# sarah-quinones/faer-rs

Hardware: AMD Instinct MI355X
Metric: achieved fp64 GFLOP/s (and % MFMA peak), GEMM + LU/Cholesky, N=16384 (higher is better)
Workload: dtype f64; 1 GPU; dgemm_f64_n8192; layout=column-major, resident in HBM

## Files before the change

faer-rs_amd/csrc/tsqr.hip:

```cpp
#include <atomic>
#include <limits>

#include "common.h"
#include "mfma.h"

namespace fh {

typedef float f32x4 __attribute__((ext_vector_type(4)));
typedef float f32x16 __attribute__((ext_vector_type(16)));
typedef double f64x4 __attribute__((ext_vector_type(4)));

constexpr int TQ_PW = 64;
constexpr int TQ_LP = 68;
constexpr int TQ_TS = 192;
constexpr int TQ_NB = 512;
constexpr int TQ_DP = 65;
constexpr double TQ_COND_MAX = 64.0 * 512.0;
constexpr double TQ_TAIL_MIN = 1e-9;
template <typename T> struct TqLim;
template <> struct TqLim<float> {
	static constexpr double eps = 1.1920928955078125e-07;
	static constexpr double cond_max = TQ_COND_MAX;
	static constexpr double sq_lo = 1e-24, sq_hi = 1e24;
};
// ... 1754 lines not shown
			tq_mm64(acc, Tm, Bm, wv, lane);
#pragma unroll
			for (int jb = 0; jb < 4; ++jb)
#pragma unroll
				for (int r = 0; r < 4; ++r) {
					const long o = (long) (16 * wv + (lane >> 4) + 4 * r) * a.ldz + c2 + 16 * jb + (lane & 15);
					Bk[o] -= acc[jb][r];
				}
		}
		__syncthreads();
	}
}

typedef double f64x2 __attribute__((ext_vector_type(2)));
constexpr int TQ_LP64 = 18;

template <typename T> struct TqVec;
template <> struct TqVec<double> {
	typedef f64x2 v;
	static constexpr int RPV = 2;
};

template <typename T> struct TqGramTArgs {
	const T *P;
	const T *X;
	long ld;
	int rows, w, t, tp;
	int nsub, nchunks;
	int want_g, want_sq;
	double *Gp;
	T *Cp;
	T *Sp;
	const int *stat;
	int c0;
	T *A1s;
};

template <typename T, bool VEC> static __device__ __forceinline__ typename TqVec<T>::v tq_ldv(const T *p, int r, int rows)
{
	constexpr int RPV = TqVec<T>::RPV;
	typename TqVec<T>::v v;
#pragma unroll
	for (int e = 0; e < RPV; ++e)
		v[e] = (T) 0;
	if (VEC && r + RPV - 1 < rows) {
		v = *reinterpret_cast<const typename TqVec<T>::v *>(p + r);
	} else {
#pragma unroll
		for (int e = 0; e < RPV; ++e)
			if (r + e < rows)
				v[e] = p[r + e];
	}
	return v;
}
template <typename T, bool VEC> static __device__ __forceinline__ void tq_stv(T *p, int r, int rows, typename TqVec<T>::v v)
{
	constexpr int RPV = TqVec<T>::RPV;
	if (VEC && r + RPV - 1 < rows) {
		*reinterpret_cast<typename TqVec<T>::v *>(p + r) = v;
	} else {
#pragma unroll
		for (int e = 0; e < RPV; ++e)
			if (r + e < rows)
				p[r + e] = v[e];
	}
}

template <typename T, int NC, bool VEC> __global__ __launch_bounds__(512, 1) void tq_gramT_kernel(const TqGramTArgs<T> a)
{
	typedef typename TqVec<T>::v vec_t;
	typedef typename Mfma<T>::acc_t cacc_t;
	constexpr int RPV = TqVec<T>::RPV;
	constexpr int SR = 8 * RPV;
	constexpr int KS = 2 * RPV;
	constexpr int LP = SR + RPV;
	static_assert(LP * sizeof(T) == TQ_LP64 * 8, "pitch");
	__shared__ T sm[2][256 * LP];
	if (tq_skip(a.stat, a.c0))
		return;
	const int tid = threadIdx.x, lane = tid & 63, wv = tid >> 6;
	const int ia = wv & 3, hf = wv >> 2;
	const int q = tid & 7, cg = tid >> 3;
	const int ncol = TQ_PW + a.tp;
	const int nslot = (ncol + 63) >> 6;
	const int nsub = a.nsub;
	const int ncolp = nslot * 64;
	f64x4 gacc[2];
	cacc_t cacc[NC > 0 ? NC : 1];
#pragma unroll
	for (int i = 0; i < 2; ++i)
		gacc[i] = f64x4{0.0, 0.0, 0.0, 0.0};
#pragma unroll
	for (int i = 0; i < (NC > 0 ? NC : 1); ++i)
#pragma unroll
		for (int r = 0; r < 4; ++r)
			cacc[i][r] = (T) 0;
	double sq[4] = {0.0, 0.0, 0.0, 0.0};
	int ldsoff[4], roff[4];
	bool act[4];
	const T *colp[4];
#pragma unroll
	for (int i = 0; i < 4; ++i) {
		const int si = i / nslot, ci = (i - si * nslot) * 64 + cg;
		const bool isp = ci < TQ_PW;
		const int cc = isp ? ci : ci - TQ_PW;
		act[i] = si < nsub && (isp ? cc < a.w : cc < a.t);
		colp[i] = act[i] ? (isp ? a.P : a.X) + (long) cc * a.ld : a.P;
		roff[i] = act[i] ? SR * si + RPV * q : RPV * q;
		ldsoff[i] = (si * ncolp + ci) * LP + RPV * q;
	}
	auto ldu = [](const T *p) {
		vec_t v;
		if (VEC) {
			v = *reinterpret_cast<const vec_t *>(p);
		} else {
#pragma unroll
			for (int x = 0; x < RPV; ++x)
				v[x] = p[x];
		}
		return v;
	};
	const int crows = SR * nsub;
	const int nfull = a.rows / crows;
	const int cpw = (nfull + (int) gridDim.x - 1) / (int) gridDim.x;
	const int first = (int) blockIdx.x * cpw;
	const int nmine = nfull - first < 0 ? 0 : (nfull - first < cpw ? nfull - first : cpw);
	if (blockIdx.x == 0 && a.want_g) {
		for (int e = tid; e < 64 * (64 / RPV); e += 512) {
			const int c = e / (64 / RPV), rp = e % (64 / RPV);
			vec_t v;
#pragma unroll
			for (int x = 0; x < RPV; ++x)
				v[x] = (T) 0;
			if (c < a.w)
				v = ldu(a.P + (long) c * a.ld + RPV * rp);
			*reinterpret_cast<vec_t *>(a.A1s + c * 64 + RPV * rp) = v;
		}
	}
	vec_t s0[4], s1[4], s2[4], s3[4];
	auto load_chunk = [&](int j, vec_t (&st)[4]) {
		const int jj = j < nmine ? j : nmine - 1;
		const long r0 = (long) (first + jj) * crows;
#pragma unroll
		for (int i = 0; i < 4; ++i)
			st[i] = ldu(colp[i] + r0 + roff[i]);
	};
	auto stage = [&](int j, const vec_t (&st)[4], double count) {
		T *dst = sm[j & 1];
#pragma unroll
		for (int i = 0; i < 4; ++i) {
			vec_t v = st[i];
			double s = 0.0;
#pragma unroll
			for (int x = 0; x < RPV; ++x) {
				v[x] = act[i] ? v[x] : (T) 0;
				s += (double) v[x] * (double) v[x];
			}
			*reinterpret_cast<vec_t *>(&dst[ldsoff[i]]) = v;
			sq[i] += count * s;
		}
	};
	auto products = [&](int j) {
		const T *src = sm[j & 1];
		const int ro = KS * (lane >> 4);
#pragma unroll 1
		for (int sb = 0; sb < nsub; ++sb) {
			const T *base = src + (long) sb * ncolp * LP + (lane & 15) * LP + ro;
			const T *ap = base + 16 * ia * LP;
			const vec_t alo = *reinterpret_cast<const vec_t *>(ap), ahi = *reinterpret_cast<const vec_t *>(ap + RPV);
#pragma unroll
			for (int c0 = 0; c0 < NC; c0 += 2) {
				vec_t blo[2], bhi[2];
#pragma unroll
				for (int c = 0; c < 2; ++c) {
					const T *bp = base + (TQ_PW + 16 * (2 * (c0 + c) + hf)) * LP;
					blo[c] = *reinterpret_cast<const vec_t *>(bp);
					bhi[c] = *reinterpret_cast<const vec_t *>(bp + RPV);
				}
#pragma unroll
				for (int x = 0; x < RPV; ++x)
#pragma unroll
					for (int c = 0; c < 2; ++c)
						cacc[c0 + c] = Mfma<T>::run(alo[x], blo[c][x], cacc[c0 + c]);
#pragma unroll
				for (int x = 0; x < RPV; ++x)
#pragma unroll
					for (int c = 0; c < 2; ++c)
						cacc[c0 + c] = Mfma<T>::run(ahi[x], bhi[c][x], cacc[c0 + c]);
			}
			if (a.want_g) {
#pragma unroll
				for (int u = 0; u < 2; ++u) {
					const int jb = 2 * hf + u;
					if (jb <= ia) {
						const T *bp = base + 16 * jb * LP;
						const vec_t glo = *reinterpret_cast<const vec_t *>(bp), ghi = *reinterpret_cast<const vec_t *>(bp + RPV);
#pragma unroll
						for (int x = 0; x < RPV; ++x)
							gacc[u] = __builtin_amdgcn_mfma_f64_16x16x4f64((double) alo[x], (double) glo[x], gacc[u], 0, 0, 0);
#pragma unroll
						for (int x = 0; x < RPV; ++x)
							gacc[u] = __builtin_amdgcn_mfma_f64_16x16x4f64((double) ahi[x], (double) ghi[x], gacc[u], 0, 0, 0);
					}
				}
			}
		}
	};
	if (nmine > 0) {
		load_chunk(0, s0);
		load_chunk(1, s1);
		load_chunk(2, s2);
		load_chunk(3, s3);
		stage(0, s0, 1.0);
		load_chunk(4, s0);
		tq_lds_barrier();
#define TQ_GT_STEP(J, SN)                                                                                                                   \
	{                                                                                                                                   \
		stage((J) + 1, SN, (J) + 1 < nmine ? 1.0 : 0.0);                                                                            \
		load_chunk((J) + 5, SN);                                                                                                    \
		products(J);                                                                                                                \
		tq_lds_barrier();                                                                                                           \
	}
		int j = 0;
#pragma unroll 1
		for (; j + 3 < nmine; j += 4) {
			TQ_GT_STEP(j, s1)
			TQ_GT_STEP(j + 1, s2)
			TQ_GT_STEP(j + 2, s3)
			TQ_GT_STEP(j + 3, s0)
		}
		if (j < nmine)
			TQ_GT_STEP(j, s1)
		if (j + 1 < nmine)
			TQ_GT_STEP(j + 1, s2)
		if (j + 2 < nmine)
			TQ_GT_STEP(j + 2, s3)
#undef TQ_GT_STEP
	}
	if (blockIdx.x == gridDim.x - 1 && nfull * crows < a.rows) {
		const long r0 = (long) nfull * crows;
#pragma unroll
		for (int i = 0; i < 4; ++i) {
#pragma unroll
			for (int x = 0; x < RPV; ++x)
				s0[i][x] = (T) 0;
			if (act[i])
				s0[i] = tq_ldv<T, VEC>(colp[i] + r0, roff[i], a.rows - (int) r0);
		}
		__syncthreads();
		stage(0, s0, 1.0);
		__syncthreads();
		products(0);
	}
	const long blk = blockIdx.x;
	if (a.want_g) {
#pragma unroll
		for (int u = 0; u < 2; ++u) {
			const int jb = 2 * hf + u;
			if (jb <= ia) {
#pragma unroll
				for (int r = 0; r < 4; ++r)
					a.Gp[blk * 4096 + (16 * ia + Mfma<double>::row(r, lane >> 4)) * 64 + 16 * jb + (lane & 15)] = gacc[u][r];
			}
		}
	}
#pragma unroll
	for (int c = 0; c < NC; ++c) {
		const int cb = 2 * c + hf;
#pragma unroll
		for (int r = 0; r < 4; ++r)
			a.Cp[blk * 64 * a.tp + (long) (16 * ia + Mfma<T>::row(r, lane >> 4)) * a.tp + 16 * cb + (lane & 15)] = cacc[c][r];
	}
	if (a.want_sq) {
		if (nslot == 1) {
			sq[0] = (sq[0] + sq[1]) + (sq[2] + sq[3]);
		} else if (nslot == 2) {
			sq[0] += sq[2];
			sq[1] += sq[3];
		}
#pragma unroll
		for (int i = 0; i < 4; ++i) {
			double v = sq[i];
			v += __shfl_xor(v, 1);
			v += __shfl_xor(v, 2);
			v += __shfl_xor(v, 4);
			if (q == 0 && i < nslot)
				a.Sp[blk * 256 + i * 64 + cg] = (T) v;
		}
	}
}

template <typename T> struct TqUpdTArgs {
	T *P;
	T *X;
	long ld;
	int rows, w, ts;
	const T *Yn;
	int typ, coff;
	const T *Mn;
	int do_v;
	int nchunks;
	const int *stat;
	int c0;
};

template <typename T, bool VEC> __global__ __launch_bounds__(512, 1) void tq_updateT_kernel(const TqUpdTArgs<T> a)
{
	typedef typename TqVec<T>::v vec_t;
	typedef typename Mfma<T>::acc_t acc_t;
	constexpr int RPV = TqVec<T>::RPV;
	constexpr int CR = 16 * RPV;
	constexpr int LPP = CR + RPV;
	__shared__ T Pl[64 * LPP];
	if (tq_skip(a.stat, a.c0))
		return;
	const int tid = threadIdx.x, lane = tid & 63, wv = tid >> 6;
	const int li = lane & 15, g = lane >> 4;
	const int nx = (a.ts + 15) >> 4;
	const int nt = nx + (a.do_v ? 4 : 0);
	T ya[2][16];
#pragma unroll
	for (int u = 0; u < 2; ++u) {
		const int tl = wv + 8 * u;
		const bool isx = tl < nx, isv = !isx && tl < nt;
		const int col = isx ? 16 * tl + li : 16 * (tl - nx) + li;
		const bool ok = isx ? col < a.ts : (isv && col < a.w);
		const T *src = isx ? a.Yn + a.coff + col : a.Mn + col;
		const long step = isx ? (long) a.typ : 64L;
#pragma unroll
		for (int ks = 0; ks < 16; ++ks)
			ya[u][ks] = ok && (4 * ks + g) < a.w ? src[(long) (4 * ks + g) * step] : (T) 0;
	}
	const int pq = tid & 15, pc = tid >> 4;
	vec_t pst[2];
	vec_t xv[2][4], xn[2][4];
	auto load_checked = [&](int ch, vec_t (&x)[2][4]) {
		const int cr = a.nchunks - 1 - ch;
		const int rb = cr * CR + RPV * pq, rbase = cr * CR + RPV * li;
#pragma unroll
		for (int i = 0; i < 2; ++i) {
			const int c = pc + 32 * i;
#pragma unroll
			for (int e = 0; e < RPV; ++e)
				pst[i][e] = (T) 0;
			if (c < a.w)
				pst[i] = tq_ldv<T, VEC>(a.P + (long) c * a.ld, rb, a.rows);
		}
#pragma unroll
		for (int u = 0; u < 2; ++u) {
			const int tl = wv + 8 * u;
#pragma unroll
			for (int r = 0; r < 4; ++r) {
#pragma unroll
				for (int e = 0; e < RPV; ++e)
					x[u][r][e] = (T) 0;
				const int col = 16 * tl + Mfma<T>::row(r, g);
				if (tl < nx && col < a.ts)
					x[u][r] = tq_ldv<T, VEC>(a.X + (long) col * a.ld, rbase, a.rows);
			}
		}
	};
	const T *pcol[2], *xcol[2][4];
#pragma unroll
	for (int i = 0; i < 2; ++i)
		pcol[i] = a.P + (long) (pc + 32 * i < a.w ? pc + 32 * i : 0) * a.ld + RPV * pq;
#pragma unroll
	for (int u = 0; u < 2; ++u)
#pragma unroll
		for (int r = 0; r < 4; ++r) {
			const int col = 16 * (wv + 8 * u) + Mfma<T>::row(r, g);
			xcol[u][r] = (a.ts > 0 ? a.X + (long) (col < a.ts ? col : a.ts - 1) * a.ld : a.P) + RPV * li;
		}
	auto load_full = [&](int ch, vec_t (&x)[2][4]) {
		const long r0 = (long) (a.nchunks - 1 - ch) * CR;
#pragma unroll
		for (int i = 0; i < 2; ++i)
			pst[i] = *reinterpret_cast<const vec_t *>(pcol[i] + r0);
#pragma unroll
		for (int u = 0; u < 2; ++u)
#pragma unroll
			for (int r = 0; r < 4; ++r)
				x[u][r] = *reinterpret_cast<const vec_t *>(xcol[u][r] + r0);
	};
	auto stage_panel = [&]() {
#pragma unroll
		for (int i = 0; i < 2; ++i) {
			vec_t v = pst[i];
#pragma unroll
			for (int e = 0; e < RPV; ++e)
				v[e] = pc + 32 * i < a.w ? v[e] : (T) 0;
			*reinterpret_cast<vec_t *>(&Pl[(pc + 32 * i) * LPP + RPV * pq]) = v;
		}
	};
	auto compute_store = [&](int ch, const vec_t (&x)[2][4]) {
		const int rbase = (a.nchunks - 1 - ch) * CR + RPV * li;
#pragma unroll
		for (int u = 0; u < 2; ++u) {
			const int tl = wv + 8 * u;
			if (tl < nt) {
				const bool isx = tl < nx;
				acc_t acc[RPV];
#pragma unroll
				for (int e = 0; e < RPV; ++e)
#pragma unroll
					for (int r = 0; r < 4; ++r)
						acc[e][r] = isx ? x[u][r][e] : (T) 0;
#pragma unroll
				for (int ks = 0; ks < 16; ++ks) {
					const vec_t b = *reinterpret_cast<const vec_t *>(&Pl[(4 * ks + g) * LPP + RPV * li]);
#pragma unroll
					for (int e = 0; e < RPV; ++e)
						acc[e] = Mfma<T>::run(ya[u][ks], b[e], acc[e]);
				}
				T *dst = isx ? a.X + (long) (16 * tl) * a.ld : a.P + (long) (16 * (tl - nx)) * a.ld;
				const int nvalid = isx ? a.ts - 16 * tl : a.w - 16 * (tl - nx);
#pragma unroll
				for (int r = 0; r < 4; ++r) {
					const int cl = Mfma<T>::row(r, g);
					vec_t o;
#pragma unroll
					for (int e = 0; e < RPV; ++e)
						o[e] = acc[e][r];
					if (cl < nvalid)
						tq_stv<T, VEC>(dst + (long) cl * a.ld, rbase, a.rows, o);
				}
			}
		}
	};
	const int cpw = (a.nchunks + (int) gridDim.x - 1) / (int) gridDim.x;
	int ch = (int) blockIdx.x * cpw;
	const int chend = ch + cpw < a.nchunks ? ch + cpw : a.nchunks;
	const int nchecked = VEC ? ((a.rows % CR) != 0 ? 1 : 0) : a.nchunks;
	for (; ch < chend && ch < nchecked; ++ch) {
		load_checked(ch, xv);
		__syncthreads();
		stage_panel();
		__syncthreads();
		compute_store(ch, xv);
	}
	if (ch >= chend)
		return;
	load_full(ch, xv);
#pragma unroll 1
	for (; ch < chend; ++ch) {
		tq_lds_barrier();
		stage_panel();
		tq_lds_barrier();
		load_full(ch + 1 < chend ? ch + 1 : ch, xn);
		compute_store(ch, xv);
#pragma unroll
		for (int u = 0; u < 2; ++u)
#pragma unroll
			for (int r = 0; r < 4; ++r)
				xv[u][r] = xn[u][r];
	}
}

static void tq_launch_form_v(bool vec, int ncu, const TqFormVArgs &va)
{
	hipStream_t s = ctx().stream;
	const int nwg = (va.nrb + 3) / 4 < ncu ? (va.nrb + 3) / 4 : ncu;
	ProfScope prof(2, (double) va.rows * 4.0 * 2.0 * (double) va.w);
	if (vec)
		hipLaunchKernelGGL(tq_form_v_kernel<true>, dim3(nwg), dim3(256), 0, s, va);
	else
		hipLaunchKernelGGL(tq_form_v_kernel<false>, dim3(nwg), dim3(256), 0, s, va);
}

static void tq_gram(const float *P, const float *X, long ld, int rows, int w, int t, bool want_g, bool want_sq, bool vec, double *Gp, float *Cp,
		    float *Sp, double *G, double *C, int ldc, int coff, double *S, const int *stat, int c0, float *A1s, double *Gf, int *cnt, int nb_max)
{
	hipStream_t s = ctx().stream;
	TqGramArgs g;
	g.A1s = A1s;
	g.P = P;
	g.X = X;
	g.ld = ld;
	g.rows = rows;
	g.w = w;
	g.t = t;
	g.tp = (t + 31) & ~31;
	g.nchunks = (rows + 63) / 64;
	g.want_g = want_g;
	g.want_sq = want_sq;
	g.Gp = Gp;
	g.Cp = Cp;
	g.Sp = Sp;
	g.stat = stat;
	g.c0 = c0;
	const int nbmax = nb_max > 0 && nb_max < TQ_NB ? nb_max : TQ_NB;
	const int nb = g.nchunks < nbmax ? g.nchunks : nbmax;
	if (nb <= 0)
		return;
	{
		ProfScope prof(3, (double) rows * 4.0 * ((double) w + (double) t));
		if (vec)
			hipLaunchKernelGGL(tq_gram_kernel<true>, dim3(nb), dim3(256), 0, s, g);
		else
			hipLaunchKernelGGL(tq_gram_kernel<false>, dim3(nb), dim3(256), 0, s, g);
	}
	const int total = (want_g ? 4096 : 0) + 64 * g.tp + (want_sq ? 256 : 0);
	hipLaunchKernelGGL(tq_reduce_kernel<float>, dim3((total + 255) / 256, TQ_NG), dim3(256), 0, s, Gp, Cp, Sp, nb, g.tp, (int) want_g, (int) want_sq, G, C,
			   ldc, coff, S, stat, c0, Gf, cnt);
	FH_HIP(hipGetLastError());
}

static std::atomic<int> g_tq_panel_copy{1};
void tsqr_debug_panel_copy(int on) { g_tq_panel_copy.store(on); }

static void tq_launch_fused(bool vec, int mode, int nwg, const TqFusedArgs &fa)
{
	hipStream_t s = ctx().stream;
	ProfScope prof(2, (double) fa.rows * 4.0 *
				  ((double) fa.w + (double) fa.wn + (mode == 1 ? (double) fa.wn + (fa.do_v ? (double) fa.w : 0.0) : 2.0 * (double) fa.ts)));
	if (mode == 1) {
		if (vec)
			hipLaunchKernelGGL((tq_fused_kernel<true, 1>), dim3(nwg), dim3(256), 0, s, fa);
		else
			hipLaunchKernelGGL((tq_fused_kernel<false, 1>), dim3(nwg), dim3(256), 0, s, fa);
	} else {
		if (vec)
			hipLaunchKernelGGL((tq_fused_kernel<true, 2>), dim3(nwg), dim3(512), 0, s, fa);
		else
			hipLaunchKernelGGL((tq_fused_kernel<false, 2>), dim3(nwg), dim3(512), 0, s, fa);
	}
}

struct TqSide {
	hipStream_t panel, tx;
	hipEvent_t pfork, pdone, xfork, xdone;
};
static TqSide tq_side()
{
	Ctx &c = ctx();
	c.qr_side_streams();
	return TqSide{c.qr_side[0], c.qr_side[1], c.qr_ev[0], c.qr_ev[1], c.qr_ev[2], c.qr_ev[3]};
}

template <typename T> __global__ __launch_bounds__(256) void tq_above_kernel(const T *A, long ld, int top, double *abv)
{
	__shared__ double red[256];
	const T *col = A + (long) blockIdx.x * ld;
	double sq = 0.0;
	for (int i = 1 + (int) threadIdx.x; i <= top; i += 256) {
		const double v = (double) col[-(long) i];
		sq += v * v;
	}
	red[threadIdx.x] = sq;
	__syncthreads();
	for (int o = 128; o > 0; o >>= 1) {
		if ((int) threadIdx.x < o)
			red[threadIdx.x] += red[threadIdx.x + o];
		__syncthreads();
	}
	if (threadIdx.x == 0)
		abv[blockIdx.x] = red[0];
}

template <typename T> __global__ __launch_bounds__(256) void tq_range_rest_kernel(const T *A, long ld, int m, int c_first, int *stat)
{
	__shared__ double red[256];
	const T *col = A + (long) (c_first + (int) blockIdx.x) * ld;
	double sq = 0.0;
	for (int i = threadIdx.x; i < m; i += 256) {
		const double v = (double) col[i];
		sq += v * v;
	}
	red[threadIdx.x] = sq;
	__syncthreads();
	for (int o = 128; o > 0; o >>= 1) {
		if ((int) threadIdx.x < o)
			red[threadIdx.x] += red[threadIdx.x + o];
		__syncthreads();
	}
	if (threadIdx.x == 0) {
		const double lo = TqLim<T>::sq_lo * (double) m, hi = TqLim<T>::sq_hi * (double) m;
		if (!(red[0] >= lo && red[0] <= hi)) {
			stat[1] = 0;
			stat[2] = TQ_FAIL_RANGE;
			__threadfence();
			atomicExch(stat, 1);
		}
	}
}

static std::atomic<long> g_tq_min_rows{1024}, g_tq_min_aspect{3};
void tsqr_debug_shape_rule(long min_rows, long min_aspect)
{
	g_tq_min_rows.store(min_rows > 0 ? min_rows : 1024);
	g_tq_min_aspect.store(min_aspect > 0 ? min_aspect : 3);
}

static std::atomic<int> g_tq_f64{1};
void tsqr_debug_f64(int on) { g_tq_f64.store(on); }
static std::atomic<int> g_tq_panels{1};
void tsqr_debug_panels(int on) { g_tq_panels.store(on); }

template <typename T> bool tsqr_applicable(MatV<T> A, idx_t bs)
{
	const idx_t m = A.nrows, n = A.ncols;
	if (sizeof(T) == 8 && g_tq_f64.load() == 0)
		return false;
	if (A.rs != 1 || A.cs < m || n < 1 || n > 512 || m < g_tq_min_rows.load() || m < g_tq_min_aspect.load() * n || m >= (1L << 30))
		return false;
	return bs % TQ_PW == 0 || TQ_PW % bs == 0;
}
template bool tsqr_applicable<float>(MatV<float>, idx_t);
template bool tsqr_applicable<double>(MatV<double>, idx_t);

template <typename T> bool tsqr_panel_applicable(idx_t m, idx_t w, idx_t rs, idx_t cs)
{
	if (g_tq_panels.load() == 0 || (sizeof(T) == 8 && g_tq_f64.load() == 0))
		return false;
	if (rs != 1 || cs < m || w < 16 || (w > TQ_PW && w != 2 * TQ_PW) || m < 256 || m < 4 * w || m >= (1L << 30))
		return false;
	return !(16.0 * (double) std::numeric_limits<T>::epsilon() * (double) m >= 1.0);
}
template bool tsqr_panel_applicable<float>(idx_t, idx_t, idx_t, idx_t);
template bool tsqr_panel_applicable<double>(idx_t, idx_t, idx_t, idx_t);

template <typename T> struct TqWork {
	MatV<T> A, H;
	T *taus;
	idx_t m = A.nrows, n = A.ncols, ld = A.cs, bs = H.nrows;
	int npan = (int) ((n + TQ_PW - 1) / TQ_PW);
	int ldc = ((int) n + 63) & ~63, typ = ldc, ldz = ldc;
	hipStream_t s = ctx().stream;
	bool cross = bs > TQ_PW && npan > 1;
	Scratch gp{(size_t) TQ_NB * 4096 * 8}, cp{(size_t) TQ_NB * 64 * TQ_TS * sizeof(T)}, sp{(size_t) TQ_NB * 256 * sizeof(T)};
	Scratch small{((size_t) TQ_NG * 4096 + 3 * 4096 + (size_t) TQ_NG * 64 * ldc + (size_t) 2 * TQ_NG * 256 + (size_t) n + 64 + (size_t) 2 * npan * 4096 +
		       (size_t) 2 * npan * 64 * ldz) * 8 +
		      ((size_t) npan * 4096 + 2 * 4096 + (size_t) 64 * typ) * sizeof(T) + 2048};
	double *G, *N1, *N3, *Gf, *C, *S, *abv, *Td, *Md, *Z, *Bx;
	T *Mn, *top, *A1s, *Yn;
	int *stat;

	TqWork(MatV<T> A_, MatV<T> H_, T *taus_, idx_t rows_above) : A(A_), H(H_), taus(taus_)
	{
		FH_CHECK(A.rs == 1, "tsqr: unit row stride");
		G = small.as<double>();
		N1 = G + (size_t) TQ_NG * 4096, N3 = N1 + 4096, Gf = N3 + 4096, C = Gf + 4096;
		S = C + (size_t) TQ_NG * 64 * ldc, abv = S + (size_t) 2 * TQ_NG * 256;
		Td = abv + n + 64, Md = Td + (size_t) npan * 4096, Z = Md + (size_t) npan * 4096, Bx = Z + (size_t) npan * 64 * ldz;
		Mn = reinterpret_cast<T *>(Bx + (size_t) npan * 64 * ldz), top = Mn + (size_t) npan * 4096, A1s = top + 4096, Yn = A1s + 4096;
		stat = reinterpret_cast<int *>(Yn + (size_t) 64 * typ);
		FH_HIP(hipMemsetAsync(stat, 0, 2048, s));
		FH_HIP(hipMemsetAsync(abv, 0, (size_t) (n + 64) * 8, s));
		if (rows_above > 0)
			hipLaunchKernelGGL(tq_above_kernel<T>, dim3((unsigned) n), dim3(256), 0, s, (const T *) A.p, (long) ld, (int) rows_above, abv);
		if (cross)
			FH_HIP(hipMemsetAsync(Z, 0, (size_t) npan * 64 * ldz * 8, s));
		if (n > TQ_PW + TQ_TS) {
			hipLaunchKernelGGL(tq_range_rest_kernel<T>, dim3((unsigned) (n - (TQ_PW + TQ_TS))), dim3(256), 0, s, A.p, (long) ld, (int) m, TQ_PW + TQ_TS, stat);
			FH_HIP(hipGetLastError());
		}
	}

	int width(int k) const { return (int) (n - k * TQ_PW < TQ_PW ? n - k * TQ_PW : TQ_PW); }

	void launch_panel(int k) const
	{
		const int c0 = k * TQ_PW, w = width(k), t = (int) n - c0 - w;
		TqPanelArgs<T> pa;
		pa.A = A.p;
		pa.ld = ld;
		pa.m = (int) m;
		pa.r0 = c0;
		pa.c0 = c0;
		pa.w = w;
		pa.n = (int) n;
		pa.G = Gf;
		pa.S = S;
		pa.check_range = k == 0;
		pa.range_cols = t < TQ_TS ? t : TQ_TS;
		pa.abv = abv;
		pa.N1 = N1;
		pa.N3 = N3;
		pa.Mn = Mn + (size_t) k * 4096;
		pa.top = top;
		pa.A1s = A1s;
		pa.Md = Md + (size_t) k * 4096;
		pa.Td = Td + (size_t) k * 4096;
		pa.H = H.p;
		pa.hrs = H.rs;
		pa.hcs = H.cs;
		pa.bs = (int) bs;
		pa.taus = taus;
		pa.stat = stat;
		pa.dbg = reinterpret_cast<long long *>(stat + 16);
		ProfScope prof(4, 1.0);
		hipLaunchKernelGGL(tq_panel_kernel<T>, dim3(1), dim3(TQ_PT), 0, s, pa);
	}

	void launch_y(int k, const double *Sr) const
	{
		const int c0 = k * TQ_PW, w = width(k), t = (int) n - c0 - w;
		if (t == 0) {
			hipLaunchKernelGGL(tq_top_kernel<T>, dim3(1), dim3(256), 0, s, A.p, (long) ld, c0, c0, w, (const T *) top, (const int *) stat);
			return;
		}
		TqYArgs<T> ya;
		ya.A = A.p;
		ya.ld = ld;
		ya.r0 = c0;
		ya.cx = c0 + w;
		ya.w = w;
		ya.t = t;
		ya.C = C;
		ya.ldc = ldc;
		ya.N1 = N1;
		ya.N3 = N3;
		ya.Md = Md + (size_t) k * 4096;
		ya.abv = abv;
		ya.Yn = Yn;
		ya.typ = typ;
		ya.Z = Z + (size_t) k * 64 * ldz;
		ya.ldz = ldz;
		ya.top = top;
		ya.stat = stat;
		ya.Sr = Sr;
		ya.check_range = k == 0;
		ya.range_cols = t < TQ_TS ? t : TQ_TS;
		ya.mrows = (int) m;
		hipLaunchKernelGGL(tq_y_kernel<T>, dim3((t + 15) / 16), dim3(256), 0, s, ya);
	}

	TqTxArgs<T> tx_args(int stage) const
	{
		TqTxArgs<T> ta;
		ta.A = A.p;
		ta.ld = ld;
		ta.n = (int) n;
		ta.bs = (int) bs;
		ta.Td = Td;
		ta.Md = Md;
		ta.Z = Z;
		ta.ldz = ldz;
		ta.B = Bx;
		ta.H = H.p;
		ta.hrs = H.rs;
		ta.hcs = H.cs;
		ta.stat = stat;
		ta.stage = stage;
		return ta;
	}

	void launch_tx_stage(const TqSide &side, int stage) const
	{
		FH_HIP(hipEventRecord(side.xfork, s));
		FH_HIP(hipStreamWaitEvent(side.tx, side.xfork, 0));
		hipLaunchKernelGGL(tq_tx_kernel<T>, dim3(npan - 1), dim3(256), 0, side.tx, tx_args(stage));
	}

	void finish_tx(const TqSide &side, bool on_side) const
	{
		if (!cross)
			return;
		if (on_side) {
			FH_HIP(hipEventRecord(side.xdone, side.tx));
			FH_HIP(hipStreamWaitEvent(s, side.xdone, 0));
		} else if (bs <= (TQ_TX_MAXL + 1) * TQ_PW) {
			hipLaunchKernelGGL(tq_tx_kernel<T>, dim3(npan - 1), dim3(256), 0, s, tx_args(0));
		} else {
			hipLaunchKernelGGL(tq_tx_general_kernel<T>, dim3(npan - 1), dim3(256), 0, s, tx_args(0));
		}
		FH_HIP(hipGetLastError());
	}

	idx_t columns_done(int *reason) const
	{
		int *st = ctx().pinned_ints();
		FH_HIP(hipMemcpyAsync(st, stat, 4 * sizeof(int), hipMemcpyDeviceToHost, s));
		FH_HIP(hipStreamSynchronize(s));
#ifdef FH_TQ_TIMING
		{
			long long d[32];
			FH_HIP(hipMemcpy(d, stat + 16, sizeof(d), hipMemcpyDeviceToHost));
			fprintf(stderr, "tq_panel phases (shader cycles): start %lld: load %lld chol %lld reload %lld lu %lld finish %lld tests %lld out %lld M %lld T %lld\n",
				d[0], d[1] - d[0], d[2] - d[1], 0LL, d[3] - d[2], d[4] - d[3], d[5] - d[4], d[6] - d[5], d[7] - d[6], d[8] - d[7]);
			fprintf(stderr, "  load: range %lld loads %lld barrier %lld fill %lld | U, U^-1, V1^-1: %lld | A iterations:", d[12] - d[0], d[13] - d[12], d[14] - d[13], d[1] - d[14], d[15] - d[3]);
			for (int i = 0; i < 7; ++i)
				fprintf(stderr, " %lld", d[17 + i] - d[16 + i]);
			fprintf(stderr, " | B iterations:");
			for (int i = 0; i < 7; ++i)
				fprintf(stderr, " %lld", d[25 + i] - d[24 + i]);
			fprintf(stderr, "\n");
			double res[3];
			memcpy(res, d + 9, sizeof(res));
			fprintf(stderr, "tq_panel residuals of the last panel: |V1 V1^-1 - I| %.3e  |U U^-1 - I| %.3e  |R~ R~^-1 - I| %.3e\n", res[0], res[1], res[2]);
		}
#endif
		*reason = st[0] ? st[2] : TQ_OK;
		return st[0] ? (idx_t) st[1] : n;
	}
};

template <> idx_t tsqr_factor<float>(MatV<float> A, MatV<float> H, float *taus, int *reason, idx_t rows_above)
{
	const TqWork<float> q(A, H, taus, rows_above);
	const idx_t m = q.m, n = q.n, ld = q.ld;
	const int npan = q.npan;
	hipStream_t s = q.s;
	const bool vec = (ld % 4 == 0) && ((uintptr_t) A.p % 16 == 0);
	const int ncu_all = ctx().stream_cus();
	int cus_taken = 0;
	auto gram_nb = [&]() { return cus_taken > 0 && ncu_all - cus_taken > 8 ? 2 * (ncu_all - cus_taken) : TQ_NB; };
	auto launch_gram = [&](int c0, int w, bool want_g, int cx, int t, bool first, double *Sd) {
		const float *P = A.p + (long) c0 * ld + c0;
		const int rows = (int) (m - c0);
		if (t == 0) {
			if (want_g)
				tq_gram(P, P, ld, rows, w, 0, true, first, vec, q.gp.as<double>(), q.cp.as<float>(), q.sp.as<float>(), q.G, q.C, q.ldc, 0, Sd, q.stat, c0, q.A1s,
					q.Gf, q.stat + 128, gram_nb());
			return;
		}
		for (int off = 0; off < t; off += TQ_TS) {
			const int ts = t - off < TQ_TS ? t - off : TQ_TS;
			tq_gram(P, A.p + (long) (cx + off) * ld + c0, ld, rows, w, ts, want_g && off == 0, first && off == 0, vec, q.gp.as<double>(), q.cp.as<float>(),
				q.sp.as<float>(), q.G, q.C, q.ldc, cx + off - (c0 + w), Sd, q.stat, c0, q.A1s, q.Gf, q.stat + 128, gram_nb());
		}
	};
	const long ldpc = (long) ((m + 63) & ~(idx_t) 63);
	const bool want_copy = g_tq_panel_copy.load() != 0 && npan > 2 && (size_t) ldpc * TQ_PW * sizeof(float) <= ((size_t) 1 << 30);
	struct OptScratch {
		void *p = nullptr;
		~OptScratch()
		{
			if (p)
				ctx().release(p);
		}
		float *f() const { return static_cast<float *>(p); }
	} pcopy;
	if (want_copy)
		pcopy.p = ctx().alloc((size_t) ldpc * TQ_PW * sizeof(float));
	const bool two_stage = q.cross && q.bs >= n && q.bs <= (TQ_TX_MAXL + 1) * TQ_PW && npan >= 2;
	const TqSide side = tq_side();
	bool tx_on_side = false;
	bool panel_on_side = false;
	double *Sy = q.S;
	if (n > TQ_PW) {
		const int w0 = TQ_PW, t0 = (int) n - TQ_PW;
		launch_gram(0, w0, true, w0, 0, true, q.S);
		FH_HIP(hipEventRecord(side.pfork, s));
		FH_HIP(hipStreamWaitEvent(side.panel, side.pfork, 0));
		cus_taken += 1;
		{
			StreamScope sc(side.panel);
			Sy = q.S + (size_t) TQ_NG * 256;
			launch_gram(0, w0, false, w0, t0, true, Sy);
			FH_HIP(hipEventRecord(side.pdone, side.panel));
		}
		q.launch_panel(0);
		panel_on_side = true;
	} else {
		launch_gram(0, (int) n, true, (int) n, 0, true, q.S);
		q.launch_panel(0);
	}
	for (int k = 0; k < npan; ++k) {
		const int c0 = k * TQ_PW;
		const int w = q.width(k);
		const int t = (int) n - c0 - w;
		const int wn = t < TQ_PW ? t : TQ_PW;
		if (panel_on_side) {
			FH_HIP(hipStreamWaitEvent(s, side.pdone, 0));
			panel_on_side = false;
			cus_taken -= 1;
		}
		q.launch_y(k, Sy);
		if (two_stage && k == npan - 1 && tx_on_side)
			q.launch_tx_stage(side, 2);
		const int r1 = c0 + w;
		const int rows = (int) (m - r1);
		const bool v2 = vec && r1 % 4 == 0;
		auto form_v = [&]() {
			if (rows <= 0)
				return;
			const TqFormVArgs va{A.p + (long) c0 * ld + r1, (long) ld, rows, w, q.Mn + (size_t) k * 4096, (rows + 127) / 128, q.stat, c0};
			tq_launch_form_v(v2, ncu_all - cus_taken > 8 ? ncu_all - cus_taken : ncu_all, va);
		};
		if (t > 0) {
			const int nchunks = (rows + 63) / 64;
			TqFusedArgs fa;
			fa.P = A.p + (long) c0 * ld + r1;
			fa.N = A.p + (long) (c0 + w) * ld + r1;
			fa.F = fa.N;
			fa.ld = ld;
			fa.ldp = ld;
			fa.rows = rows;
			fa.w = w;
			fa.wn = wn;
			fa.ts = 0;
			fa.upd_n = 1;
			const bool copyp = t - wn > 0 && pcopy.p;
			fa.do_v = t - wn == 0 || copyp;
			fa.Pc = copyp ? pcopy.f() : nullptr;
			fa.ldpc = ldpc;
			fa.want_g = 1;
			fa.Yn = q.Yn;
			fa.typ = q.typ;
			fa.fo = 0;
			fa.Mn = q.Mn + (size_t) k * 4096;
			fa.Gp = q.gp.as<double>();
			fa.Cp = q.cp.as<float>();
			fa.tp = 0;
			fa.nchunks = nchunks;
			fa.A1s = q.A1s;
			fa.stat = q.stat;
			fa.c0 = c0;
			auto grid = [&]() {
				const int ncu = ncu_all - cus_taken > 8 ? ncu_all - cus_taken : ncu_all;
				return nchunks < 2 * ncu ? nchunks : 2 * ncu;
			};
			const int nc0 = c0 + w;
			int nb = grid();
			tq_launch_fused(v2, 1, nb, fa);
			hipLaunchKernelGGL(tq_reduce_kernel<float>, dim3(4096 / 256, TQ_NG), dim3(256), 0, s, fa.Gp, fa.Cp, q.sp.as<float>(), nb, 0, 1, 0, q.G, q.C, q.ldc, 0, q.S, q.stat, nc0,
					   q.Gf, q.stat + 128);
			if (t - wn > 0) {
				FH_HIP(hipEventRecord(side.pfork, s));
				FH_HIP(hipStreamWaitEvent(side.panel, side.pfork, 0));
				cus_taken += 1;
				{
					StreamScope sc(side.panel);
					fa.upd_n = 0;
					fa.want_g = 0;
					fa.do_v = 0;
					if (copyp) {
						fa.P = pcopy.f();
						fa.ldp = ldpc;
					}
					for (int fo = 0; fo < t - wn; fo += TU_CF) {
						fa.ts = t - wn - fo < TU_CF ? t - wn - fo : TU_CF;
						fa.tp = (fa.ts + 31) & ~31;
						fa.fo = fo;
						fa.F = A.p + (long) (nc0 + wn + fo) * ld + r1;
						nb = grid();
						tq_launch_fused(v2, 2, nb, fa);
						hipLaunchKernelGGL(tq_reduce_kernel<float>, dim3((64 * fa.tp + 255) / 256, TQ_NG), dim3(256), 0, side.panel, fa.Gp, fa.Cp, q.sp.as<float>(), nb,
								   fa.tp, 0, 0, q.G, q.C, q.ldc, fo, q.S, q.stat, nc0, q.Gf, q.stat + 128);
					}
					FH_HIP(hipEventRecord(side.pdone, side.panel));
					if (!copyp)
						form_v();
				}
				panel_on_side = true;
			}
			if (two_stage && k == npan - 2) {
				q.launch_tx_stage(side, 1);
				tx_on_side = true;
				if (ncu_all > 8 * npan)
					cus_taken += npan - 1;
			}
			q.launch_panel(k + 1);
		} else {
			form_v();
		}
		FH_HIP(hipGetLastError());
	}
	q.finish_tx(side, tx_on_side);
	if (npan > 1) {
		FH_HIP(hipEventRecord(side.pdone, side.panel));
		FH_HIP(hipStreamWaitEvent(s, side.pdone, 0));
	}
	return q.columns_done(reason);
}

template <> idx_t tsqr_factor<double>(MatV<double> A, MatV<double> H, double *taus, int *reason, idx_t rows_above)
{
	const TqWork<double> q(A, H, taus, rows_above);
	const idx_t m = q.m, n = q.n, ld = q.ld;
	const int npan = q.npan;
	hipStream_t s = q.s;
	constexpr int RPV = TqVec<double>::RPV;
	const bool vec = ld % RPV == 0 && (uintptr_t) A.p % 16 == 0;
	const int ncu = ctx().stream_cus();
	auto launch_gram = [&](int c0, int w, int cx, int t, bool first) {
		const int rows = (int) (m - c0);
		const int nstrip = t == 0 ? 1 : (t + TQ_TS - 1) / TQ_TS;
		for (int st = 0; st < nstrip; ++st) {
			const int off = st * TQ_TS;
			TqGramTArgs<double> g;
			g.P = A.p + (long) c0 * ld + c0;
			g.X = A.p + (long) (cx + off) * ld + c0;
			g.ld = ld;
			g.rows = rows;
			g.w = w;
			g.t = t - off < TQ_TS ? t - off : TQ_TS;
			g.tp = (g.t + 63) & ~63;
			{
				const int nslot = (TQ_PW + g.tp + 63) / 64;
				g.nsub = 4 / nslot;
			}
			g.nchunks = (rows + 8 * RPV * g.nsub - 1) / (8 * RPV * g.nsub);
			g.want_g = st == 0;
			g.want_sq = first && st == 0;
			g.Gp = q.gp.as<double>();
			g.Cp = q.cp.as<double>();
			g.Sp = q.sp.as<double>();
			g.stat = q.stat;
			g.c0 = c0;
			g.A1s = q.A1s;
			const int nb = g.nchunks < ncu ? g.nchunks : ncu;
			{
				ProfScope prof(3, (double) rows * 8.0 * ((double) w + (double) g.t));
				switch (g.tp / 32) {
				case 0: if (vec)
						hipLaunchKernelGGL((tq_gramT_kernel<double, 0, true>), dim3(nb), dim3(512), 0, s, g);
					else
						hipLaunchKernelGGL((tq_gramT_kernel<double, 0, false>), dim3(nb), dim3(512), 0, s, g); break;
				case 2: if (vec)
						hipLaunchKernelGGL((tq_gramT_kernel<double, 2, true>), dim3(nb), dim3(512), 0, s, g);
					else
						hipLaunchKernelGGL((tq_gramT_kernel<double, 2, false>), dim3(nb), dim3(512), 0, s, g); break;
				case 4: if (vec)
						hipLaunchKernelGGL((tq_gramT_kernel<double, 4, true>), dim3(nb), dim3(512), 0, s, g);
					else
						hipLaunchKernelGGL((tq_gramT_kernel<double, 4, false>), dim3(nb), dim3(512), 0, s, g); break;
				default: if (vec)
						hipLaunchKernelGGL((tq_gramT_kernel<double, 6, true>), dim3(nb), dim3(512), 0, s, g);
					else
						hipLaunchKernelGGL((tq_gramT_kernel<double, 6, false>), dim3(nb), dim3(512), 0, s, g); break;
				}
			}
			const int total = (g.want_g ? 4096 : 0) + 64 * g.tp + (g.want_sq ? 256 : 0);
			hipLaunchKernelGGL(tq_reduce_kernel<double>, dim3((total + 255) / 256, TQ_NG), dim3(256), 0, s, g.Gp, g.Cp, g.Sp, nb, g.tp, g.want_g, g.want_sq, q.G, q.C, q.ldc,
					   cx + off - (c0 + w), q.S, q.stat, c0, q.Gf, q.stat + 128);
			FH_HIP(hipGetLastError());
		}
	};
	const bool two_stage = q.cross && q.bs >= n && q.bs <= (TQ_TX_MAXL + 1) * TQ_PW && npan >= 2;
	const TqSide side = tq_side();
	for (int k = 0; k < npan; ++k) {
		const int c0 = k * TQ_PW;
		const int w = q.width(k);
		const int t = (int) n - c0 - w;
		if (two_stage && k == npan - 1)
			q.launch_tx_stage(side, 1);
		launch_gram(c0, w, c0 + w, t, k == 0);
		q.launch_panel(k);
		q.launch_y(k, q.S);
		if (two_stage && k == npan - 1)
			q.launch_tx_stage(side, 2);
		const int r1 = c0 + w;
		const int rows = (int) (m - r1);
		if (rows > 0) {
			TqUpdTArgs<double> ua;
			ua.P = A.p + (long) c0 * ld + r1;
			ua.ld = ld;
			ua.rows = rows;
			ua.w = w;
			ua.Yn = q.Yn;
			ua.typ = q.typ;
			ua.Mn = q.Mn + (size_t) k * 4096;
			ua.nchunks = (rows + 16 * RPV - 1) / (16 * RPV);
			ua.stat = q.stat;
			ua.c0 = c0;
			const bool v2 = vec && r1 % RPV == 0;
			const int nwg = ua.nchunks < ncu ? ua.nchunks : ncu;
			int from = 0;
			do {
				int ts = t - from;
				const bool last = ts <= TQ_TS;
				if (!last)
					ts = TQ_TS;
				ua.coff = from;
				ua.ts = ts;
				ua.X = A.p + (long) (c0 + w + from) * ld + r1;
				ua.do_v = last;
				ProfScope prof(2, (double) rows * 8.0 * ((double) w + 2.0 * (double) ts + (last ? (double) w : 0.0)));
				if (v2)
					hipLaunchKernelGGL((tq_updateT_kernel<double, true>), dim3(nwg), dim3(512), 0, s, ua);
				else
					hipLaunchKernelGGL((tq_updateT_kernel<double, false>), dim3(nwg), dim3(512), 0, s, ua);
				from += ts;
				if (last)
					break;
			} while (true);
		}
		FH_HIP(hipGetLastError());
	}
	q.finish_tx(side, two_stage);
	return q.columns_done(reason);
}

}
```

Before: 72270 GFLOP/s.

## Fuse next-panel Gram computation into trailing update kernel for fp64 TSQR

The trailing-update kernel for the first strip now also computes the Gram matrix and cross products for the next panel. It stages the freshly updated columns in LDS and accumulates MFMA products there, so the next step no longer has to launch a separate Gram pass that re-reads those columns from HBM. Only the remaining strips beyond the first still use the standalone gram launch. The change costs extra LDS, more registers in a launch_bounds(512,1) kernel, a partial-sum reduce launch, and a reshuffled prefetch and barrier schedule, which could lower overlap or affect correctness.

```diff
diff --git a/faer-rs_amd/csrc/tsqr.hip b/faer-rs_amd/csrc/tsqr.hip
--- a/faer-rs_amd/csrc/tsqr.hip
+++ b/faer-rs_amd/csrc/tsqr.hip
@@ -2080,20 +2080,42 @@
 	int nchunks;
 	const int *stat;
 	int c0;
+	int wn, tp;
+	double *Gp;
+	T *Cp;
+	T *A1s;
 };
 
-template <typename T, bool VEC> __global__ __launch_bounds__(512, 1) void tq_updateT_kernel(const TqUpdTArgs<T> a)
+template <typename T, bool VEC, bool GRAM> __global__ __launch_bounds__(512, 1) void tq_updateT_kernel(const TqUpdTArgs<T> a)
 {
 	typedef typename TqVec<T>::v vec_t;
 	typedef typename Mfma<T>::acc_t acc_t;
 	constexpr int RPV = TqVec<T>::RPV;
 	constexpr int CR = 16 * RPV;
 	constexpr int LPP = CR + RPV;
+	constexpr int XC = GRAM ? TQ_PW + 128 : 1;
 	__shared__ T Pl[64 * LPP];
+	__shared__ T Xl[XC * LPP];
 	if (tq_skip(a.stat, a.c0))
 		return;
 	const int tid = threadIdx.x, lane = tid & 63, wv = tid >> 6;
 	const int li = lane & 15, g = lane >> 4;
+	const int ia = wv & 3, hf = wv >> 2;
+	const int ncf = GRAM ? a.tp >> 5 : 0;
+	f64x4 gacc[2];
+	acc_t cacc[4];
+	if (GRAM) {
+#pragma unroll
+		for (int i = 0; i < 2; ++i)
+			gacc[i] = f64x4{0.0, 0.0, 0.0, 0.0};
+#pragma unroll
+		for (int i = 0; i < 4; ++i)
+#pragma unroll
+			for (int r = 0; r < 4; ++r)
+				cacc[i][r] = (T) 0;
+		for (int e = tid; e < XC * LPP; e += 512)
+			Xl[e] = (T) 0;
+	}
 	const int nx = (a.ts + 15) >> 4;
 	const int nt = nx + (a.do_v ? 4 : 0);
 	T ya[2][16];
@@ -2170,8 +2192,9 @@
 			*reinterpret_cast<vec_t *>(&Pl[(pc + 32 * i) * LPP + RPV * pq]) = v;
 		}
 	};
-	auto compute_store = [&](int ch, const vec_t (&x)[2][4]) {
-		const int rbase = (a.nchunks - 1 - ch) * CR + RPV * li;
+	auto compute_store = [&](int ch, vec_t (&x)[2][4], long rnext) {
+		const int cr = a.nchunks - 1 - ch;
+		const int rbase = cr * CR + RPV * li;
 #pragma unroll
 		for (int u = 0; u < 2; ++u) {
 			const int tl = wv + 8 * u;
@@ -2183,6 +2206,11 @@
 #pragma unroll
 					for (int r = 0; r < 4; ++r)
 						acc[e][r] = isx ? x[u][r][e] : (T) 0;
+				if (GRAM && rnext >= 0) {
+#pragma unroll
+					for (int r = 0; r < 4; ++r)
+						x[u][r] = *reinterpret_cast<const vec_t *>(xcol[u][r] + rnext);
+				}
 #pragma unroll
 				for (int ks = 0; ks < 16; ++ks) {
 					const vec_t b = *reinterpret_cast<const vec_t *>(&Pl[(4 * ks + g) * LPP + RPV * li]);
@@ -2201,9 +2229,53 @@
 						o[e] = acc[e][r];
 					if (cl < nvalid)
 						tq_stv<T, VEC>(dst + (long) cl * a.ld, rbase, a.rows, o);
+					if (GRAM && isx) {
+						if (cl >= nvalid) {
+#pragma unroll
+							for (int e = 0; e < RPV; ++e)
+								o[e] = (T) 0;
+						}
+						*reinterpret_cast<vec_t *>(&Xl[(16 * tl + cl) * LPP + RPV * li]) = o;
+						if (cr < 64 / CR && 16 * tl + cl < a.wn)
+							*reinterpret_cast<vec_t *>(a.A1s + (16 * tl + cl) * 64 + cr * CR + RPV * li) = o;
+					}
 				}
 			}
 		}
+	};
+	auto gram_products = [&]() {
+		constexpr int KS = CR / 4, NV = KS / RPV;
+		const T *base = Xl + (lane & 15) * LPP + KS * (lane >> 4);
+		vec_t av[NV], bv[NV];
+#pragma unroll
+		for (int v = 0; v < NV; ++v)
+			av[v] = *reinterpret_cast<const vec_t *>(base + 16 * ia * LPP + RPV * v);
+#pragma unroll
+		for (int c = 0; c < 4; ++c)
+			if (c < ncf) {
+				const T *bp = base + (TQ_PW + 16 * (2 * c + hf)) * LPP;
+#pragma unroll
+				for (int v = 0; v < NV; ++v)
+					bv[v] = *reinterpret_cast<const vec_t *>(bp + RPV * v);
+#pragma unroll
+				for (int v = 0; v < NV; ++v)
+#pragma unroll
+					for (int x = 0; x < RPV; ++x)
+						cacc[c] = Mfma<T>::run(av[v][x], bv[v][x], cacc[c]);
+			}
+#pragma unroll
+		for (int u = 0; u < 2; ++u)
+			if (2 * hf + u <= ia) {
+				const T *bp = base + 16 * (2 * hf + u) * LPP;
+#pragma unroll
+				for (int v = 0; v < NV; ++v)
+					bv[v] = *reinterpret_cast<const vec_t *>(bp + RPV * v);
+#pragma unroll
+				for (int v = 0; v < NV; ++v)
+#pragma unroll
+					for (int x = 0; x < RPV; ++x)
+						gacc[u] = __builtin_amdgcn_mfma_f64_16x16x4f64((double) av[v][x], (double) bv[v][x], gacc[u], 0, 0, 0);
+			}
 	};
 	const int cpw = (a.nchunks + (int) gridDim.x - 1) / (int) gridDim.x;
 	int ch = (int) blockIdx.x * cpw;
@@ -2214,23 +2286,57 @@
 		__syncthreads();
 		stage_panel();
 		__syncthreads();
-		compute_store(ch, xv);
-	}
-	if (ch >= chend)
-		return;
-	load_full(ch, xv);
+		compute_store(ch, xv, -1);
+		if (GRAM) {
+			__syncthreads();
+			gram_products();
+		}
+	}
+	if (ch < chend) {
+		load_full(ch, xv);
 #pragma unroll 1
-	for (; ch < chend; ++ch) {
-		tq_lds_barrier();
-		stage_panel();
-		tq_lds_barrier();
-		load_full(ch + 1 < chend ? ch + 1 : ch, xn);
-		compute_store(ch, xv);
+		for (; ch < chend; ++ch) {
+			if (!GRAM)
+				tq_lds_barrier();
+			stage_panel();
+			tq_lds_barrier();
+			const int nxt = ch + 1 < chend ? ch + 1 : ch;
+			if (GRAM) {
+				const long rnext = (long) (a.nchunks - 1 - nxt) * CR;
+#pragma unroll
+				for (int i = 0; i < 2; ++i)
+					pst[i] = *reinterpret_cast<const vec_t *>(pcol[i] + rnext);
+				compute_store(ch, xv, rnext);
+				tq_lds_barrier();
+				gram_products();
+			} else {
+				load_full(nxt, xn);
+				compute_store(ch, xv, -1);
+#pragma unroll
+				for (int u = 0; u < 2; ++u)
+#pragma unroll
+					for (int r = 0; r < 4; ++r)
+						xv[u][r] = xn[u][r];
+			}
+		}
+	}
+	if (GRAM) {
+		const long blk = blockIdx.x;
+		const int gi = lane & 15, gq = lane >> 4;
 #pragma unroll
 		for (int u = 0; u < 2; ++u)
-#pragma unroll
-			for (int r = 0; r < 4; ++r)
-				xv[u][r] = xn[u][r];
+			if (2 * hf + u <= ia) {
+#pragma unroll
+				for (int r = 0; r < 4; ++r)
+					a.Gp[blk * 4096 + (16 * ia + Mfma<double>::row(r, gq)) * 64 + 16 * (2 * hf + u) + gi] = gacc[u][r];
+			}
+#pragma unroll
+		for (int c = 0; c < 4; ++c)
+			if (c < ncf) {
+#pragma unroll
+				for (int r = 0; r < 4; ++r)
+					a.Cp[blk * 64 * a.tp + (long) (16 * ia + Mfma<T>::row(r, gq)) * a.tp + 16 * (2 * c + hf) + gi] = cacc[c][r];
+			}
 	}
 }
 
@@ -2752,7 +2858,7 @@
 	constexpr int RPV = TqVec<double>::RPV;
 	const bool vec = ld % RPV == 0 && (uintptr_t) A.p % 16 == 0;
 	const int ncu = ctx().stream_cus();
-	auto launch_gram = [&](int c0, int w, int cx, int t, bool first) {
+	auto launch_gram = [&](int c0, int w, int cx, int t, bool first, bool with_g, int step) {
 		const int rows = (int) (m - c0);
 		const int nstrip = t == 0 ? 1 : (t + TQ_TS - 1) / TQ_TS;
 		for (int st = 0; st < nstrip; ++st) {
@@ -2770,13 +2876,13 @@
 				g.nsub = 4 / nslot;
 			}
 			g.nchunks = (rows + 8 * RPV * g.nsub - 1) / (8 * RPV * g.nsub);
-			g.want_g = st == 0;
+			g.want_g = with_g && st == 0;
 			g.want_sq = first && st == 0;
 			g.Gp = q.gp.as<double>();
 			g.Cp = q.cp.as<double>();
 			g.Sp = q.sp.as<double>();
 			g.stat = q.stat;
-			g.c0 = c0;
+			g.c0 = step;
 			g.A1s = q.A1s;
 			const int nb = g.nchunks < ncu ? g.nchunks : ncu;
 			{
@@ -2802,19 +2908,20 @@
 			}
 			const int total = (g.want_g ? 4096 : 0) + 64 * g.tp + (g.want_sq ? 256 : 0);
 			hipLaunchKernelGGL(tq_reduce_kernel<double>, dim3((total + 255) / 256, TQ_NG), dim3(256), 0, s, g.Gp, g.Cp, g.Sp, nb, g.tp, g.want_g, g.want_sq, q.G, q.C, q.ldc,
-					   cx + off - (c0 + w), q.S, q.stat, c0, q.Gf, q.stat + 128);
+					   cx + off - (c0 + w), q.S, q.stat, step, q.Gf, q.stat + 128);
 			FH_HIP(hipGetLastError());
 		}
 	};
 	const bool two_stage = q.cross && q.bs >= n && q.bs <= (TQ_TX_MAXL + 1) * TQ_PW && npan >= 2;
 	const TqSide side = tq_side();
+	launch_gram(0, q.width(0), q.width(0), (int) n - q.width(0), true, true, 0);
 	for (int k = 0; k < npan; ++k) {
 		const int c0 = k * TQ_PW;
 		const int w = q.width(k);
 		const int t = (int) n - c0 - w;
+		const int wn = t < TQ_PW ? t : TQ_PW;
 		if (two_stage && k == npan - 1)
 			q.launch_tx_stage(side, 1);
-		launch_gram(c0, w, c0 + w, t, k == 0);
 		q.launch_panel(k);
 		q.launch_y(k, q.S);
 		if (two_stage && k == npan - 1)
@@ -2833,6 +2940,10 @@
 			ua.nchunks = (rows + 16 * RPV - 1) / (16 * RPV);
 			ua.stat = q.stat;
 			ua.c0 = c0;
+			ua.wn = wn;
+			ua.Gp = q.gp.as<double>();
+			ua.Cp = q.cp.as<double>();
+			ua.A1s = q.A1s;
 			const bool v2 = vec && r1 % RPV == 0;
 			const int nwg = ua.nchunks < ncu ? ua.nchunks : ncu;
 			int from = 0;
@@ -2845,15 +2956,31 @@
 				ua.ts = ts;
 				ua.X = A.p + (long) (c0 + w + from) * ld + r1;
 				ua.do_v = last;
-				ProfScope prof(2, (double) rows * 8.0 * ((double) w + 2.0 * (double) ts + (last ? (double) w : 0.0)));
-				if (v2)
-					hipLaunchKernelGGL((tq_updateT_kernel<double, true>), dim3(nwg), dim3(512), 0, s, ua);
-				else
-					hipLaunchKernelGGL((tq_updateT_kernel<double, false>), dim3(nwg), dim3(512), 0, s, ua);
+				const bool gram = from == 0 && t > 0;
+				ua.tp = (ts - wn + 31) & ~31;
+				{
+					ProfScope prof(2, (double) rows * 8.0 * ((double) w + 2.0 * (double) ts + (last ? (double) w : 0.0)));
+					if (gram) {
+						if (v2)
+							hipLaunchKernelGGL((tq_updateT_kernel<double, true, true>), dim3(nwg), dim3(512), 0, s, ua);
+						else
+							hipLaunchKernelGGL((tq_updateT_kernel<double, false, true>), dim3(nwg), dim3(512), 0, s, ua);
+					} else {
+						if (v2)
+							hipLaunchKernelGGL((tq_updateT_kernel<double, true, false>), dim3(nwg), dim3(512), 0, s, ua);
+						else
+							hipLaunchKernelGGL((tq_updateT_kernel<double, false, false>), dim3(nwg), dim3(512), 0, s, ua);
+					}
+				}
+				if (gram)
+					hipLaunchKernelGGL(tq_reduce_kernel<double>, dim3((4096 + 64 * ua.tp + 255) / 256, TQ_NG), dim3(256), 0, s, ua.Gp, ua.Cp, q.sp.as<double>(), nwg,
+							   ua.tp, 1, 0, q.G, q.C, q.ldc, 0, q.S, q.stat, c0, q.Gf, q.stat + 128);
 				from += ts;
 				if (last)
 					break;
 			} while (true);
+			if (t > TQ_TS)
+				launch_gram(r1, wn, r1 + TQ_TS, t - TQ_TS, false, false, c0);
 		}
 		FH_HIP(hipGetLastError());
 	}
```

Result: no change. 72190 GFLOP/s (median of 3 runs) (-0.1%).
